# Kateridge/TransMF_AD

Measured on AMD Instinct MI355X. Metric: volume-pairs/sec fwd+bwd(+Adam), 96^3 MRI+PET batch=8 per GPU, higher is better.
Workload: dtype f32

## Files before the change

transmf_ad_amd/csrc/conv3d_wino.hip:

```cpp
#include <type_traits>
#include "tmf_device.h"

namespace {

constexpr int TD = 4, TH = 8, TW = 8;
constexpr int CK = 8;
constexpr int NTHR = 512;
constexpr int GROUPS = 768, SLOTS = 2 * GROUPS;
constexpr int RAW_BYTES = SLOTS * 16;
constexpr int NDMA = SLOTS / NTHR;
constexpr int B_OFF = 2 * RAW_BYTES;
constexpr int B_BYTES = 8 * 8 * 64 * 16;
constexpr int EX_FLOATS = 8 * 8 * 2 * 64 * 4;
constexpr int RED_OFF = EX_FLOATS;
constexpr int LDS_FLOATS = RED_OFF + 8 * 32 * 2;
constexpr size_t LDS_BYTES = (size_t)LDS_FLOATS * 4;
static_assert(B_OFF + B_BYTES <= EX_FLOATS * 4, "LDS carving");

__device__ __forceinline__ constexpr int ogd(int dd) { return (dd & 1) * 384 + (dd >> 1) * 32; }
__device__ __forceinline__ constexpr int ogh(int i) { return (i & 1) * 192 + (i >> 1) * 6; }
__device__ __forceinline__ constexpr int ogw(int k) { return (k & 1) * 96 + (k >> 1); }

#ifdef TMF_WINO_TRACE
__device__ long long g_wino_blocks[8192 * 4];
// ... 863 lines not shown
constexpr int WX_SLOTS = 3072, WX_REAL = 360 * 8, WZ_SLOTS = 1024;
constexpr int WBUF_BYTES = (WX_SLOTS + WZ_SLOTS) * 16;
constexpr int WZ_OFF = WX_SLOTS * 4;
constexpr size_t WG_LDS_BYTES = 2 * (size_t)WBUF_BYTES;

__global__ __launch_bounds__(NTHR) void conv3d_wino_wgrad_kernel(
    const float* __restrict__ x, const float* __restrict__ dz, float* __restrict__ partial,
    int D, int H, int W, int Cin, int Cout, int tilesD, int tilesH, int tilesW, int nbricks, int per_split, int ncob) {
    extern __shared__ __attribute__((aligned(16))) float smem[];
    const unsigned lds0 = (unsigned)(size_t)(__attribute__((address_space(3))) const void*)smem;
    const int tid = threadIdx.x;
    const int lane = tid & 63;
    const int wave = __builtin_amdgcn_readfirstlane(tid >> 6);
    const int l31 = lane & 31, hsel = lane >> 5;
    const int split = blockIdx.x, blk = blockIdx.y;
    const int ci0 = (blk / ncob) * 32, co0 = (blk % ncob) * 32;
    const int st0 = split * per_split;
    const int st1 = st0 + per_split < nbricks ? st0 + per_split : nbricks;
    constexpr int OOB = (int)0x80000000u;

    int relx[6], pcx[6], relz[2], pcz[2];
#pragma unroll
    for (int q = 0; q < 6; ++q) {
        const int e = (q * 8 + wave) * 64 + lane, v = e >> 3, piece = e & 7;
        const int hd = v / 60, hh = (v / 10) % 6, hw = v % 10;
        relx[q] = (((hd - 1) * H + (hh - 1)) * W + (hw - 1)) * Cin * 4 + piece * 16;
        pcx[q] = e < WX_REAL ? (hd | (hh << 8) | (hw << 16)) : -1;
    }
#pragma unroll
    for (int q = 0; q < 2; ++q) {
        const int e = (q * 8 + wave) * 64 + lane, v = e >> 3, piece = e & 7;
        const int od = v >> 5, oh = (v >> 3) & 3, ow = v & 7;
        relz[q] = ((od * H + oh) * W + ow) * Cout * 4 + piece * 16;
        pcz[q] = od | (oh << 8) | (ow << 16);
    }
    auto stage = [&](int st) {
        int t = st;
        const int bw = t % tilesW; t /= tilesW;
        const int bh = t % tilesH; t /= tilesH;
        const int bd = t % tilesD;
        const int b = t / tilesD;
        const int d0 = bd * 4, h0 = bh * 4, w0 = bw * 8;
        const i32x4 xr = make_rsrc(x + (size_t)b * D * H * W * Cin, (unsigned)(D * H * W * Cin * 4));
        const i32x4 zr = make_rsrc(dz + (size_t)b * D * H * W * Cout, (unsigned)(D * H * W * Cout * 4));
        const int xbase = ((d0 * H + h0) * W + w0) * Cin * 4 + ci0 * 4, zbase = ((d0 * H + h0) * W + w0) * Cout * 4 + co0 * 4;
        const unsigned base = lds0 + ((st - st0) & 1) * WBUF_BYTES + wave * 1024;
#pragma unroll
        for (int q = 0; q < 6; ++q) {
            const int hd = pcx[q] & 255, hh = (pcx[q] >> 8) & 255, hw = (pcx[q] >> 16) & 255;
            const bool ok = pcx[q] >= 0 && (unsigned)(d0 - 1 + hd) < (unsigned)D && (unsigned)(h0 - 1 + hh) < (unsigned)H &&
                            (unsigned)(w0 - 1 + hw) < (unsigned)W;
            blds16(ok ? relx[q] + xbase : OOB, xr, 0, base + q * 8192);
        }
#pragma unroll
        for (int q = 0; q < 2; ++q) {
            const int od = pcz[q] & 255, oh = (pcz[q] >> 8) & 255, ow = (pcz[q] >> 16) & 255;
            const bool ok = d0 + od < D && h0 + oh < H && w0 + ow < W;
            blds16(ok ? relz[q] + zbase : OOB, zr, 0, base + WX_SLOTS * 16 + q * 8192);
        }
    };

    const int mpd = wave >> 1, mhh = wave & 1;
    const int da = mpd == 0 ? 0 : (mpd == 2 ? 2 : 1);
    const int db = mpd == 0 ? 2 : (mpd == 1 ? 2 : (mpd == 2 ? 1 : 3));
    const float sgn = mpd == 1 ? 1.f : -1.f;
    const int ik = mhh == 0 ? 2 : 1, ia = mhh == 0 ? 0 : 2, ib = mhh == 0 ? 1 : 3;
    const float c1 = mhh == 0 ? 1.f : -1.f;
    const float ca = mpd == 3 ? 0.f : 1.f, cb = mpd == 0 ? 0.f : (mpd == 1 ? 1.f : -1.f);
    const float e0 = mhh == 0 ? 0.f : -1.f, f0 = mhh == 0 ? 1.f : 0.f, f1 = mhh == 0 ? 1.f : -1.f;
    const int lx = l31 + hsel * 64;
    auto xrow = [&](int dd, int i) { return lx + (dd * 60 + i * 10) * 32; };
    const int rka = xrow(da, ik), rkb = xrow(db, ik), raa = xrow(da, ia), rab = xrow(db, ia), rba = xrow(da, ib), rbb = xrow(db, ib);
    const int lz = WZ_OFF + l31 + hsel * 64;

    f32x16 acc[8];
#pragma unroll
    for (int q = 0; q < 8; ++q)
#pragma unroll
        for (int r = 0; r < 16; ++r) acc[q][r] = 0.f;

    if (st0 < st1) {
        stage(st0);
        vm_wait<0>();
        __syncthreads();
    }
    for (int st = st0; st < st1; ++st) {
        if (st + 1 < st1) stage(st + 1);
        const float* R = smem + ((st - st0) & 1) * (WBUF_BYTES / 4);
#pragma unroll
        for (int j = 0; j < 8; ++j) {
            const int td = j >> 2, th = (j >> 1) & 1, twb = (j & 1) * 2;
            const int xo = ((2 * td * 6 + 2 * th) * 10 + 2 * twb) * 32, zo = ((2 * td * 4 + 2 * th) * 8 + 2 * twb) * 32;
            auto wrow = [&](int pa, int pb, float (&wv)[4]) {
                float tv[4];
#pragma unroll
                for (int k = 0; k < 4; ++k) tv[k] = R[pa + xo + k * 32] + sgn * R[pb + xo + k * 32];
                wv[0] = tv[0] - tv[2]; wv[1] = tv[1] + tv[2]; wv[2] = tv[2] - tv[1]; wv[3] = tv[1] - tv[3];
            };
            float wk[4], A0[4], A1[4];
            wrow(rka, rkb, wk);
            wrow(raa, rab, A0);
            wrow(rba, rbb, A1);
#pragma unroll
            for (int k = 0; k < 4; ++k) {
                A0[k] = A0[k] - wk[k];
                A1[k] = c1 * A1[k] + wk[k];
            }
            float u[2][2];
#pragma unroll
            for (int wo = 0; wo < 2; ++wo) {
                float zd[2];
#pragma unroll
                for (int ho = 0; ho < 2; ++ho)
                    zd[ho] = ca * R[lz + zo + ((0 * 4 + ho) * 8 + wo) * 32] + cb * R[lz + zo + ((1 * 4 + ho) * 8 + wo) * 32];
                u[0][wo] = zd[0] + e0 * zd[1];
                u[1][wo] = f0 * zd[0] + f1 * zd[1];
            }
#pragma unroll
            for (int phl = 0; phl < 2; ++phl) {
                const float b0 = u[phl][0], b1 = u[phl][0] + u[phl][1], b2 = u[phl][0] - u[phl][1], b3 = -u[phl][1];
                const float* Ap = phl == 0 ? A0 : A1;
                acc[phl * 4 + 0] = __builtin_amdgcn_mfma_f32_32x32x2f32(Ap[0], b0, acc[phl * 4 + 0], 0, 0, 0);
                acc[phl * 4 + 1] = __builtin_amdgcn_mfma_f32_32x32x2f32(Ap[1], b1, acc[phl * 4 + 1], 0, 0, 0);
                acc[phl * 4 + 2] = __builtin_amdgcn_mfma_f32_32x32x2f32(Ap[2], b2, acc[phl * 4 + 2], 0, 0, 0);
                acc[phl * 4 + 3] = __builtin_amdgcn_mfma_f32_32x32x2f32(Ap[3], b3, acc[phl * 4 + 3], 0, 0, 0);
            }
        }
        vm_wait<0>();
        __syncthreads();
    }

    float* out = partial + (((size_t)split * gridDim.y + blk) * 64 + (mpd * 16 + mhh * 8)) * 1024;
#pragma unroll
    for (int q = 0; q < 8; ++q)
#pragma unroll
        for (int r = 0; r < 16; ++r)
            out[q * 1024 + ((r & 3) + 8 * (r >> 2) + 4 * hsel) * 32 + l31] = acc[q][r];
}

template <int C, int PAIR = 2>
__device__ __forceinline__ f32x2 lds_pair(unsigned base_even, unsigned base_odd) {
    f32x2 d;
    asm volatile("ds_read2st64_b32 %0, %1 offset0:%2 offset1:%3" : "=v"(d) : "v"((C & 1) ? base_odd : base_even), "n"(C >> 1), "n"((C >> 1) + PAIR));
    return d;
}
__device__ __forceinline__ void lds_wait() { asm volatile("s_waitcnt lgkmcnt(0)" ::: "memory"); }
template <int N, typename F>
__device__ __forceinline__ void static_for(F&& f) {
    if constexpr (N > 0) {
        static_for<N - 1>(f);
        f(std::integral_constant<int, N - 1>{});
    }
}
constexpr int WPN = 256;
template <int GEOM> struct WGeomP {
    static constexpr int ROWW = GEOM == 0 ? 10 : 12, PLANE = 6 * ROWW, PAIR = GEOM == 0 ? 2 : 3, BW = GEOM == 0 ? 8 : 4, BS = GEOM == 0 ? 1 : 2;
    static constexpr int XREAL = 36 * ROWW * 8;
    static constexpr int XDMA = (XREAL + 4 * 64 - 1) / (4 * 64);
    static constexpr int XSLOTS = XDMA * WPN;
    static constexpr int BUF_BYTES = (XSLOTS + WZ_SLOTS) * 16;
    static constexpr size_t LDS_BYTES = 2 * (size_t)BUF_BYTES;
};
constexpr int WP_ZDMA = WZ_SLOTS / WPN;

template <int GEOM>
__global__ __launch_bounds__(WPN) void conv3d_wino_wgrad_p_kernel(
    const float* __restrict__ x, const float* __restrict__ dz, float* __restrict__ partial,
    int B, int D, int H, int W, int Cin, int Cout, int tilesD, int tilesH, int tilesW, int nbricks, int per_split, int ncob) {
    using WG = WGeomP<GEOM>;
    constexpr int WP_XDMA = WG::XDMA, WX_SLOTS = WG::XSLOTS, WX_REAL = WG::XREAL, WBUF_BYTES = WG::BUF_BYTES;
    constexpr int ROWW = WG::ROWW, PLANE = WG::PLANE, PAIR = WG::PAIR;
    extern __shared__ __attribute__((aligned(16))) float smem[];
    const unsigned lds0 = (unsigned)(size_t)(__attribute__((address_space(3))) const void*)smem;
    const int tid = threadIdx.x;
    const int lane = tid & 63;
    const int wave = __builtin_amdgcn_readfirstlane(tid >> 6);
    const int l31 = lane & 31, hsel = lane >> 5;
    const int split = xcd_contiguous(blockIdx.x, gridDim.x), blk = blockIdx.y;
    const int ci0 = (blk / ncob) * 32, co0 = (blk % ncob) * 32;
    const int st0 = split * per_split;
    const int st1 = st0 + per_split < nbricks ? st0 + per_split : nbricks;
    constexpr int OOB = (int)0x80000000u;

    int relx[WP_XDMA], mx[WP_XDMA], relz[WP_ZDMA], mz[WP_ZDMA];
#pragma unroll
    for (int q = 0; q < WP_XDMA; ++q) {
        const int e = (q * 4 + wave) * 64 + lane, v = e >> 3, piece = e & 7;
        const int hd = v / PLANE, hh = (v / ROWW) % 6, hr = v % ROWW, s_ = GEOM == 0 ? 0 : hr / 6, hw = GEOM == 0 ? hr : hr % 6;
        relx[q] = (((s_ * D + hd) * H + hh) * W + hw) * Cin * 4 + piece * 16;
        mx[q] = e < WX_REAL ? (1 << hd) | (1 << (8 + hh)) | (1 << (16 + hw)) | (1 << (26 + s_)) : (1 << 30);
    }
#pragma unroll
    for (int q = 0; q < WP_ZDMA; ++q) {
        const int e = (q * 4 + wave) * 64 + lane, v = e >> 3, piece = e & 7;
        const int od = v >> 5, oh = (v >> 3) & 3, s_ = GEOM == 0 ? 0 : (v >> 2) & 1, ow = GEOM == 0 ? v & 7 : v & 3;
        relz[q] = (((s_ * D + od) * H + oh) * W + ow) * Cout * 4 + piece * 16;
        mz[q] = (1 << od) | (1 << (8 + oh)) | (1 << (16 + ow)) | (1 << (26 + s_));
    }
    int sbw = 0, sbh = 0, sbd = 0, sb = 0;
    auto stage_first = [&](int st) {
        int t = st;
        sbw = t % tilesW; t /= tilesW;
        sbh = t % tilesH; t /= tilesH;
        sbd = t % tilesD;
        sb = t / tilesD;
    };
    auto stage_next = [&]() {
        if (++sbw == tilesW) { sbw = 0; if (++sbh == tilesH) { sbh = 0; if (++sbd == tilesD) { sbd = 0; ++sb; } } }
    };
    i32x4 s_xr, s_zr;
    int s_xcorner = 0, s_zcorner = 0, s_vmx = 0, s_vmz = 0;
    unsigned s_base = 0;
    auto stage_setup = [&](int buf) {
        const int b = sb * WG::BS, d0 = sbd * 4, h0 = sbh * 4, w0 = sbw * WG::BW;
        const int ns = B - b < WG::BS ? B - b : WG::BS;
        s_xr = make_rsrc(x + (size_t)b * D * H * W * Cin, (unsigned)(ns * D * H * W * Cin * 4));
        s_zr = make_rsrc(dz + (size_t)b * D * H * W * Cout, (unsigned)(ns * D * H * W * Cout * 4));
        s_xcorner = (((d0 - 1) * H + (h0 - 1)) * W + (w0 - 1)) * Cin * 4 + ci0 * 4;
        s_zcorner = ((d0 * H + h0) * W + w0) * Cout * 4 + co0 * 4;
        auto range = [](int lo, int hi) { return ((1 << hi) - 1) & ~((1 << lo) - 1); };
        auto mn = [](int a, int b_) { return a < b_ ? a : b_; };
        s_vmx = range(d0 == 0 ? 1 : 0, mn(6, D - d0 + 1)) | (range(h0 == 0 ? 1 : 0, mn(6, H - h0 + 1)) << 8) |
                (range(w0 == 0 ? 1 : 0, mn(WG::BW + 2, W - w0 + 1)) << 16) | (range(0, ns) << 26);
        s_vmz = range(0, mn(4, D - d0)) | (range(0, mn(4, H - h0)) << 8) | (range(0, mn(WG::BW, W - w0)) << 16) | (range(0, ns) << 26);
        s_base = lds0 + buf * WBUF_BYTES + wave * 1024;
    };
    auto stage_part = [&](int part) {
        if (P_ABL & 4) return;
#pragma unroll
        for (int q = 0; q < WP_XDMA; ++q)
            if (q * 3 / WP_XDMA == part) blds16((mx[q] & s_vmx) == mx[q] ? relx[q] + s_xcorner : OOB, s_xr, 0, s_base + q * 4096);
#pragma unroll
        for (int q = 0; q < WP_ZDMA; ++q)
            if (3 == part) blds16((mz[q] & s_vmz) == mz[q] ? relz[q] + s_zcorner : OOB, s_zr, 0, s_base + WX_SLOTS * 16 + q * 4096);
    };
    auto stage_issue = [&](int buf) {
        stage_setup(buf);
#pragma unroll
        for (int i = 0; i < 4; ++i) stage_part(i);
    };

    const int da = wave == 0 ? 0 : (wave == 2 ? 2 : 1);
    const int db = wave == 0 ? 2 : (wave == 1 ? 2 : (wave == 2 ? 1 : 3));
    const float sgn = wave == 1 ? 1.f : -1.f;
    const f32x2 s2 = {sgn, sgn};
    const float cz = wave == 1 ? 1.f : (wave == 2 ? -1.f : 0.f);
    const f32x2 cz2 = {cz, cz};
    const unsigned zfirst = wave == 3 ? 4 * 8 * 32 * 4 : 0;
    const unsigned lx = lds0 + (2 * hsel * 32 + l31) * 4;
    const unsigned xa0 = lx + da * PLANE * 128, xb0 = lx + db * PLANE * 128, zz0 = lx + WX_SLOTS * 16;
    f32x2 A[16], Bv[16];
#if P_ABL & 1
    for (int i = 0; i < 16; ++i) { A[i] = f32x2{(float)tid, 1.f}; Bv[i] = f32x2{(float)lane, 2.f}; }
#endif
    f32x2 u1[4], u2[4], zd[2][2];
    f32x16 acc[16];
#pragma unroll
    for (int q = 0; q < 16; ++q)
#pragma unroll
        for (int r = 0; r < 16; ++r) acc[q][r] = 0.f;

    auto pin4 = [](f32x2& a, f32x2& b, f32x2& c, f32x2& d) { asm volatile("" : "+v"(a), "+v"(b), "+v"(c), "+v"(d)); };
    f32x2 ra[4], rb[4];
    auto row_issue = [&](unsigned ea, unsigned eb, auto c_c) {
        constexpr int Cb = decltype(c_c)::value;
        static_for<4>([&](auto k_c) {
            constexpr int K = decltype(k_c)::value;
            ra[K] = lds_pair<Cb + K, PAIR>(ea, ea + 128);
            rb[K] = lds_pair<Cb + K, PAIR>(eb, eb + 128);
        });
    };
    auto row_finish = [&](f32x2 (&u)[4]) {
        lds_wait();
        pin4(ra[0], ra[1], ra[2], ra[3]);
        pin4(rb[0], rb[1], rb[2], rb[3]);
        pk_row4(u, ra, rb, s2);
    };
    auto zrows = [&](f32x2 ya0, f32x2 ya1, int pha, f32x2 yb0, f32x2 yb1, int phb) {
        Bv[pha * 4 + 0] = ya0; Bv[pha * 4 + 3] = ya1; Bv[phb * 4 + 0] = yb0; Bv[phb * 4 + 3] = yb1;
        pk_z2(Bv[pha * 4 + 1], Bv[pha * 4 + 2], Bv[phb * 4 + 1], Bv[phb * 4 + 2], ya0, ya1, yb0, yb1);
    };
    f32x2 yq[2][2][2];
    f32x2 v0[4];
    auto T1 = [&](int par, auto step_c, int part) {
        constexpr int STEP = decltype(step_c)::value, TDs = STEP >> 1, THs = STEP & 1;
        if (P_ABL & 1) return;
        const unsigned off = par * WBUF_BYTES;
        if (part == 0) {
            row_issue(xa0 + off, xb0 + off, std::integral_constant<int, (2 * TDs) * PLANE + (2 * THs + 1) * ROWW>{});
            static_for<2>([&](auto ho_c) {
                static_for<2>([&](auto wo_c) {
                    constexpr int HO = decltype(ho_c)::value, WO = decltype(wo_c)::value;
                    constexpr int C0 = ((2 * TDs + 0) * 4 + (2 * THs + HO)) * 8 + WO, C1 = ((2 * TDs + 1) * 4 + (2 * THs + HO)) * 8 + WO;
                    yq[0][HO][WO] = lds_pair<C0>(zz0 + zfirst + off, zz0 + zfirst + off + 128);
                    yq[1][HO][WO] = lds_pair<C1>(zz0 + off, zz0 + off + 128);
                });
            });
        } else if (part == 1) {
            row_finish(u1);
            pin4(yq[0][0][0], yq[0][0][1], yq[0][1][0], yq[0][1][1]);
            pin4(yq[1][0][0], yq[1][0][1], yq[1][1][0], yq[1][1][1]);
            row_issue(xa0 + off, xb0 + off, std::integral_constant<int, (2 * TDs) * PLANE + (2 * THs + 2) * ROWW>{});
#pragma unroll
            for (int ho = 0; ho < 2; ++ho)
#pragma unroll
                for (int wo = 0; wo < 2; ++wo) zd[ho][wo] = pk_fma(cz2, yq[1][ho][wo], yq[0][ho][wo]);
            {
                f32x2 zs0, zdf0, zs1, zdf1;
                pk_z2(zs0, zdf0, zs1, zdf1, zd[0][0], zd[1][0], zd[0][1], zd[1][1]);
                zrows(zs0, zs1, 1, zdf0, zdf1, 2);
            }
            pin4(u1[0], u1[1], u1[2], u1[3]);
            pin4(Bv[4], Bv[5], Bv[6], Bv[7]); pin4(Bv[8], Bv[9], Bv[10], Bv[11]);
        } else {
            row_finish(u2);
            {
                f32x2 sm[4], df[4];
                pk_addsub4(sm, df, u2, u1);
#pragma unroll
                for (int k = 0; k < 4; ++k) { A[4 + k] = sm[k]; A[8 + k] = df[k]; }
            }
            pin4(A[4], A[5], A[6], A[7]); pin4(A[8], A[9], A[10], A[11]);
        }
    };
    auto T2 = [&](int par, auto step_c, int part) {
        constexpr int STEP = decltype(step_c)::value, TDs = STEP >> 1, THs = STEP & 1;
        if (P_ABL & 1) return;
        const unsigned off = par * WBUF_BYTES;
        if (part == 0) {
            row_issue(xa0 + off, xb0 + off, std::integral_constant<int, (2 * TDs) * PLANE + (2 * THs + 0) * ROWW>{});
            zrows(zd[0][0], zd[0][1], 0, zd[1][0], zd[1][1], 3);
            pin4(Bv[0], Bv[1], Bv[2], Bv[3]); pin4(Bv[12], Bv[13], Bv[14], Bv[15]);
        } else if (part == 1) {
            row_finish(v0);
            row_issue(xa0 + off, xb0 + off, std::integral_constant<int, (2 * TDs) * PLANE + (2 * THs + 3) * ROWW>{});
            {
                f32x2 d[4];
                pk_sub4(d, v0, u2);
#pragma unroll
                for (int k = 0; k < 4; ++k) A[k] = d[k];
            }
            pin4(A[0], A[1], A[2], A[3]);
        } else {
            row_finish(v0);
            {
                f32x2 d[4];
                pk_sub4(d, u1, v0);
#pragma unroll
                for (int k = 0; k < 4; ++k) A[12 + k] = d[k];
            }
            pin4(A[12], A[13], A[14], A[15]);
        }
    };
    auto mfma_g = [&](int pha, int phb, int g) {
        const int k0 = g == 2 ? 0 : 2 * g, k1 = g == 2 ? 4 : 2 * g + 2, s0 = g == 2 ? 1 : 0;
#pragma unroll
        for (int k = k0; k < k1; ++k) {
#if P_ABL & 16
            acc[pha * 4 + k][s0] += A[pha * 4 + k][s0] * Bv[pha * 4 + k][s0]; acc[phb * 4 + k][s0] += A[phb * 4 + k][s0] * Bv[phb * 4 + k][s0];
#else
            acc[pha * 4 + k] = __builtin_amdgcn_mfma_f32_32x32x2f32(A[pha * 4 + k][s0], Bv[pha * 4 + k][s0], acc[pha * 4 + k], 0, 0, 0);
            acc[phb * 4 + k] = __builtin_amdgcn_mfma_f32_32x32x2f32(A[phb * 4 + k][s0], Bv[phb * 4 + k][s0], acc[phb * 4 + k], 0, 0, 0);
#endif
        }
    };

    if (st0 < st1) {
        stage_first(st0);
        stage_issue(0);
        if (st0 + 1 < st1) { stage_next(); stage_issue(1); }
        vm_wait<0>();
        __syncthreads();
#pragma unroll
        for (int g = 0; g < 3; ++g) T1(0, std::integral_constant<int, 0>{}, g);
        bool pend = false;
        for (int st = st0; st < st1; ++st) {
            const int par = (st - st0) & 1;
            static_for<4>([&](auto step_c) {
                constexpr int STEP = decltype(step_c)::value;
                __builtin_amdgcn_sched_barrier(0);
                if (STEP < 2 && pend) { stage_part(1 + 2 * STEP); if (STEP == 1) pend = false; }
#pragma unroll
                for (int g = 0; g < 3; ++g) {
                    __builtin_amdgcn_sched_barrier(0);
                    T2(par, step_c, g);
                    mfma_g(1, 2, g);
                }
                __builtin_amdgcn_sched_barrier(0);
                if (STEP == 3) {
                    vm_wait<0>();
                    __syncthreads();
                    if (st + 2 < st1) { stage_next(); stage_setup(par); stage_part(0); pend = true; }
                }
                if (STEP == 0 && pend) stage_part(2);
#pragma unroll
                for (int g = 0; g < 3; ++g) {
                    __builtin_amdgcn_sched_barrier(0);
                    T1(STEP < 3 ? par : par ^ 1, std::integral_constant<int, (STEP + 1) & 3>{}, g);
                    mfma_g(0, 3, g);
                }
                __builtin_amdgcn_sched_barrier(0);
            });
        }
    }

    __syncthreads();
    float* slab = partial + (size_t)split * 27 * Cin * Cout + (size_t)ci0 * Cout + co0 + l31;
    auto gt3 = [](float u0, float u1, float u2, float u3, float (&o)[3]) {
        const float sm = u1 + u2, df = u1 - u2;
        o[0] = u0 + 0.5f * sm; o[1] = 0.5f * df; o[2] = 0.5f * sm - u3;
    };
#pragma unroll
    for (int half = 0; half < 2; ++half) {
#pragma unroll
        for (int rr = 0; rr < 8; ++rr) {
            const int r = half * 8 + rr;
            float t[4][3], v[3][3];
#pragma unroll
            for (int ph = 0; ph < 4; ++ph)
                gt3(acc_read(acc[ph * 4 + 0][r]), acc_read(acc[ph * 4 + 1][r]), acc_read(acc[ph * 4 + 2][r]), acc_read(acc[ph * 4 + 3][r]), t[ph]);
#pragma unroll
            for (int j = 0; j < 3; ++j) {
                float o[3];
                gt3(t[0][j], t[1][j], t[2][j], t[3][j], o);
                v[0][j] = o[0]; v[1][j] = o[1]; v[2][j] = o[2];
            }
#pragma unroll
            for (int i = 0; i < 3; ++i)
#pragma unroll
                for (int j = 0; j < 3; ++j) smem[((wave * 8 + rr) * 9 + i * 3 + j) * 64 + lane] = v[i][j];
            __builtin_amdgcn_sched_barrier(0);
        }
        __syncthreads();
#pragma unroll
        for (int q = 0; q < 18; ++q) {
            const int e = wave * 18 + q, rr = e / 9, ij = e % 9;
            float V[4], o[3];
#pragma unroll
            for (int pd = 0; pd < 4; ++pd) V[pd] = smem[((pd * 8 + rr) * 9 + ij) * 64 + lane];
            gt3(V[0], V[1], V[2], V[3], o);
            const int r = half * 8 + rr, ci = (r & 3) + 8 * (r >> 2) + 4 * hsel;
#pragma unroll
            for (int kd = 0; kd < 3; ++kd) slab[((size_t)(kd * 9 + ij) * Cin + ci) * Cout] = o[kd];
        }
        __syncthreads();
    }
}

__global__ __launch_bounds__(256) void wino_wgrad_finish_kernel(const float* __restrict__ du, float* __restrict__ dw,
                                                                int cin, int cout, int ncob, int dw_ref) {
    const int e = blockIdx.x * 256 + threadIdx.x;
    if (e >= cin * cout) return;
    const int co = e % cout, ci = e / cout;
    const int blk = (ci / 32) * ncob + co / 32;
    const float* src = du + (size_t)blk * 64 * 1024 + (ci % 32) * 32 + (co % 32);
    double u[4][4][4];
#pragma unroll
    for (int p = 0; p < 4; ++p)
#pragma unroll
        for (int q = 0; q < 4; ++q)
#pragma unroll
            for (int r = 0; r < 4; ++r) u[p][q][r] = (double)src[((p * 4 + q) * 4 + r) * 1024];
    auto GT = [](double u0, double u1, double u2, double u3, int a) {
        return a == 0 ? u0 + 0.5 * (u1 + u2) : (a == 1 ? 0.5 * (u1 - u2) : 0.5 * (u1 + u2) + u3);
    };
    double t1[3][4][4], t2[3][3][4];
#pragma unroll
    for (int a = 0; a < 3; ++a)
#pragma unroll
        for (int q = 0; q < 4; ++q)
#pragma unroll
            for (int r = 0; r < 4; ++r) t1[a][q][r] = GT(u[0][q][r], u[1][q][r], u[2][q][r], u[3][q][r], a);
#pragma unroll
    for (int a = 0; a < 3; ++a)
#pragma unroll
        for (int bq = 0; bq < 3; ++bq)
#pragma unroll
            for (int r = 0; r < 4; ++r) t2[a][bq][r] = GT(t1[a][0][r], t1[a][1][r], t1[a][2][r], t1[a][3][r], bq);
#pragma unroll
    for (int a = 0; a < 3; ++a)
#pragma unroll
        for (int bq = 0; bq < 3; ++bq)
#pragma unroll
            for (int c = 0; c < 3; ++c) {
                const float v = (float)GT(t2[a][bq][0], t2[a][bq][1], t2[a][bq][2], t2[a][bq][3], c);
                const int tap = (a * 3 + bq) * 3 + c;
                if (dw_ref) dw[((size_t)co * cin + ci) * 27 + tap] = v;
                else dw[((size_t)tap * cin + ci) * cout + co] = v;
            }
}

int wino_p_mode();
struct WinoWgPlan { int geom, tilesD, tilesH, tilesW, nbricks, nblk, ncob, nsplit, per; };
WinoWgPlan plan_wino_wgrad(int B, int D, int H, int W, int cin, int cout) {
    WinoWgPlan p;
    p.tilesD = tmf_cdiv(D, 4); p.tilesH = tmf_cdiv(H, 4); p.tilesW = tmf_cdiv(W, 8);
    p.nbricks = B * p.tilesD * p.tilesH * p.tilesW;
    p.geom = 0;
    const long two = 2L * D * H * W * (cin > cout ? cin : cout) * 4;
    const int nb1 = tmf_cdiv(B, 2) * p.tilesD * p.tilesH * tmf_cdiv(W, 4);
    if (wino_p_mode() && nb1 < p.nbricks && two < (1L << 31)) {
        p.geom = 1;
        p.tilesW = tmf_cdiv(W, 4);
        p.nbricks = nb1;
// ... 397 lines not shown
```

transmf_ad_amd/csrc/conv3d_winox.hip:

```cpp
#include <type_traits>
#include "tmf_device.h"

#ifndef X_PF
#define X_PF 2
#endif
#ifndef X_NGFAST
#define X_NGFAST 1
#endif
#ifndef X_SKEW
#define X_SKEW 0
#endif
#ifndef X_RB
#define X_RB 0
#endif
#ifndef X_ABL
#define X_ABL 0
#endif

namespace {

#ifdef TMF_WINOX_TRACE
__device__ long long g_winox_phases[8 * 64];
#define XTR(i) do { __builtin_amdgcn_sched_barrier(0); if (blockIdx.x == 77 && it == 1 && lane == 0) xtr_lds[wave * 64 + (i)] = (long long)__builtin_readcyclecounter(); __builtin_amdgcn_sched_barrier(0); } while (0)
#define XTRC(i) XTR((i) + 20 * (c & 1))
#else
#define XTR(i)
#define XTRC(i)
#endif

constexpr int XN = 512;
constexpr int XCK = 16;
constexpr int BD = 4, BH = 8, BW = 8;
constexpr int CP = 96, SD = 32, SH = 6;
constexpr int SLOTS_G = 16 * CP;
constexpr int RAWB = SLOTS_G * 16;
constexpr int XDMA = SLOTS_G / XN;
constexpr int TS = 68;
constexpr int EX_OFF = 2 * RAWB;
constexpr int EX_BYTES = 8 * 32 * TS * 4;
constexpr int RED_OFF = EX_OFF + EX_BYTES;
constexpr int PLAN_OFF = RED_OFF + 2 * 64 * 33 * 4 + 64;
constexpr int TAB_OFF = PLAN_OFF + 9 * XN * 4;
#ifdef TMF_WINOX_TRACE
constexpr int TAB = 96;
#else
constexpr int TAB = 256;
#endif
constexpr size_t X_LDS_BYTES = (size_t)TAB_OFF + 256 * 32;
static_assert(EX_OFF + EX_BYTES >= 4 * RAWB && X_LDS_BYTES <= 160 * 1024, "LDS carving");

__device__ __forceinline__ void pin3(i32x4& a, i32x4& b, i32x4& c) { asm volatile("" : "+v"(a), "+v"(b), "+v"(c)); }
__device__ __forceinline__ void wg_barrier() {
    asm volatile("s_waitcnt lgkmcnt(0)\n\ts_barrier" ::: "memory");
}

__device__ __forceinline__ void wg_barrier_if(int flag) {
    asm volatile("s_cmp_eq_u32 %0, 0\n\ts_cbranch_scc1 .LWGB%=\n\ts_waitcnt lgkmcnt(0)\n\ts_barrier\n.LWGB%=:" ::"s"(__builtin_amdgcn_readfirstlane(flag)) : "memory", "scc");
}

__device__ __forceinline__ void split8(const float (&y0)[4], const float (&y1)[4], i32x4& H, i32x4& M, i32x4& L) {
#pragma unroll
    for (int j = 0; j < 4; ++j) {
        const float a = j < 2 ? y0[2 * j] : y1[2 * j - 4], b = j < 2 ? y0[2 * j + 1] : y1[2 * j - 3];
        const unsigned ua = __builtin_bit_cast(unsigned, a), ub = __builtin_bit_cast(unsigned, b);
        const float ra = a - __builtin_bit_cast(float, ua & 0xFFFF0000u), rb = b - __builtin_bit_cast(float, ub & 0xFFFF0000u);
        const unsigned va = __builtin_bit_cast(unsigned, ra), vb = __builtin_bit_cast(unsigned, rb);
        const float la = ra - __builtin_bit_cast(float, va & 0xFFFF0000u), lb = rb - __builtin_bit_cast(float, vb & 0xFFFF0000u);
        H[j] = (int)__builtin_amdgcn_perm(ub, ua, 0x07060302u);
        M[j] = (int)__builtin_amdgcn_perm(vb, va, 0x07060302u);
        L[j] = (int)__builtin_amdgcn_perm(__builtin_bit_cast(unsigned, lb), __builtin_bit_cast(unsigned, la), 0x07060302u);
    }
}
__device__ __forceinline__ f32x16 mfma_bf16(i32x4 a, i32x4 b, f32x16 c) {
    return __builtin_amdgcn_mfma_f32_32x32x16_bf16(__builtin_bit_cast(tmf_bf16x8, a), __builtin_bit_cast(tmf_bf16x8, b), c, 0, 0, 0);
}

template <int MODE>
__global__ __launch_bounds__(XN) void conv3d_winox_kernel(
    const float* __restrict__ x, const unsigned short* __restrict__ u3, float* __restrict__ z, float* __restrict__ stat_partial,
    int B, int D, int H, int W, int Cin, int Cout, int tilesD, int tilesH, int tilesW, int nbricks, int item0, int nitems,
    int stat_rows, int stat_accum, const float* __restrict__ aff_scale = nullptr, const float* __restrict__ aff_shift = nullptr,
    float slope = 0.f, int swap = 0) {
    const int sd = swap ? W : H * W, sh = swap ? D * W : W;
    constexpr bool STATS = MODE == 1;
    constexpr bool AFFINE = MODE >= 2, POOL = MODE == 3;
    constexpr int EPI_STORES = POOL ? 1 : 4;
    extern __shared__ __attribute__((aligned(16))) float smem[];
    float* ex = smem + EX_OFF / 4;
    float* red = smem + RED_OFF / 4;
    i32x4* tab = reinterpret_cast<i32x4*>(smem + TAB_OFF / 4);
#ifdef TMF_WINOX_TRACE
    long long* xtr_lds = reinterpret_cast<long long*>(smem + TAB_OFF / 4 + TAB * 8);
    for (int i = threadIdx.x; i < 512; i += XN) xtr_lds[i] = 0;
#endif
    const unsigned lds0 = (unsigned)(size_t)(__attribute__((address_space(3))) const void*)smem;
    const int tid = threadIdx.x;
    const int lane = tid & 63;
    const int wave = __builtin_amdgcn_readfirstlane(tid >> 6);
    const int l31 = lane & 31, hsel = lane >> 5;
    const int mpd = wave >> 1, mhh = wave & 1;
    const int late = (X_SKEW && wave >= 4) ? 1 : 0, early = late ^ 1;
    const int nchunk = Cin / XCK;
    constexpr int OOB = (int)0x80000000u;

    const int G = gridDim.x;
    const int jb = xcd_contiguous(blockIdx.x, G);
    const int my_items = jb < nitems ? (nitems - jb + G - 1) / G : 0;
    if (my_items == 0) return;
    for (int i = tid; i < my_items; i += XN) {
        const int item = item0 + jb + i * G;
#if X_NGFAST
        const int ngroups = Cout >> 5;
        int t = item / ngroups;
        const int ng = item - t * ngroups;
#else
        const int ng = item / nbricks;
        int t = item - ng * nbricks;
#endif
        const int bw = t % tilesW; t /= tilesW;
        const int bh = t % tilesH; t /= tilesH;
        const int bd = t % tilesD;
        const int b0 = t / tilesD;
        tab[2 * i] = i32x4{0, ng, b0, bd | (bh << 10) | (bw << 20)};
        const int d0 = bd * BD, h0 = bh * BH, w0 = bw * BW;
        auto range = [](int lo, int hi) { return ((1 << hi) - 1) & ~((1 << lo) - 1); };
        auto mn = [](int a, int b_) { return a < b_ ? a : b_; };
        tab[2 * i + 1] = i32x4{((d0 - 1) * sd + (h0 - 1) * sh + (w0 - 1)) * Cin * 4,
                               range(d0 == 0 ? 1 : 0, mn(BD + 2, D - d0 + 1)) | (range(h0 == 0 ? 1 : 0, mn(BH + 2, H - h0 + 1)) << 6) |
                                   (range(w0 == 0 ? 1 : 0, mn(BW + 2, W - w0 + 1)) << 16), 0, 0};
    }
    __syncthreads();

    int* plan = reinterpret_cast<int*>(smem + PLAN_OFF / 4) + tid;
#pragma unroll
    for (int q = 0; q < XDMA; ++q) {
        const int e = (q * 8 + wave) * 64 + lane, gg = e >> 1, par = gg / CP, g = gg % CP;
        const int a_ = g / 32, bb = (g % 32) / 6, c_ = (g % 32) % 6;
        const bool real = bb < 5 && c_ < 5;
        const int hd = 2 * a_ + (par >> 2), hh = 2 * bb + ((par >> 1) & 1), hw = 2 * c_ + (par & 1);
        const int quad = (e & 1) ^ (bb & 1);
        plan[q * XN] = ((hd * sd + hh * sh + hw) * Cin + quad * 4) * 4;
        plan[(3 + q) * XN] = real ? (1 << hd) | (1 << (6 + hh)) | (1 << (16 + hw)) : (1 << 30);
    }
    i32x4 xr = make_rsrc(x, 0);
    int dm_i = 0, dm_c = 0;
    auto dma_plan = [&](int i) {
        int corner = 0, vm = 0;
        if (i >= 0) {
            const i32x4 e1 = tab[2 * i + 1];
            const int b = __builtin_amdgcn_readfirstlane(tab[2 * i][2]);
            corner = __builtin_amdgcn_readfirstlane(e1[0]);
            vm = __builtin_amdgcn_readfirstlane(e1[1]);
            xr = make_rsrc(x + (size_t)b * D * H * W * Cin, (unsigned)(D * H * W * Cin * 4));
        }
#pragma unroll
        for (int q = 0; q < XDMA; ++q) {
            const int m = plan[(3 + q) * XN];
            plan[(6 + q) * XN] = (m & vm) == m ? plan[q * XN] + corner : OOB;
        }
    };
    auto dma_part = [&](int pr, int part) {
        const unsigned base = lds0 + pr * 2 * RAWB + wave * 1024 + part * 8192;
        const int ho = plan[(6 + part) * XN];
        if (!(X_ABL & 4)) {
            blds16_uniform(ho, xr, dm_c * (XCK * 4), base);
            blds16_uniform(ho, xr, dm_c * (XCK * 4) + 32, base + RAWB);
// ... 57 lines not shown
        for (int k = 0; k < 4; ++k) {
#pragma unroll
            for (int e = 0; e < 4; ++e) {
                const float tx = ax[k][e] + sgn * bx[k][e], tk = ak[k][e] + sgn * bk[k][e];
                T[k][e] = GA ? tx - tk : c1 * tx + tk;
            }
        }
#pragma unroll
        for (int e = 0; e < 4; ++e) {
            Y[0][e] = T[0][e] - T[2][e]; Y[1][e] = T[1][e] + T[2][e]; Y[2][e] = T[2][e] - T[1][e]; Y[3][e] = T[1][e] - T[3][e];
        }
    };

    f32x16 acc[8];

    const int r_td = wave >> 2, r_th = wave & 3;
    auto lane_now = [&]() { int l = lane; asm volatile("" : "+v"(l)); return l; };
    int st_n0 = -1;
    unsigned st_seen = 0;
    auto stat_zero = [&]() {
        const int le = lane_now();
        float* red_l = red + (wave * 8 + (le >> 3)) * 33 + 4 * (le & 7);
#pragma unroll
        for (int e = 0; e < 4; ++e) { red_l[e] = 0.f; red_l[64 * 33 + e] = 0.f; }
    };
    auto stat_flush = [&]() {
        __syncthreads();
        if (tid < 256) {
            const int part = tid & 3, ch = (tid >> 2) & 31, which = tid >> 7;
            float a = 0.f;
#pragma unroll
            for (int m = 0; m < 16; ++m) a += red[(which * 64 + part * 16 + m) * 33 + ch];
            a += __builtin_bit_cast(float, __builtin_amdgcn_mov_dpp(__builtin_bit_cast(int, a), 0xB1, 0xF, 0xF, true));
            a += __builtin_bit_cast(float, __builtin_amdgcn_mov_dpp(__builtin_bit_cast(int, a), 0x4E, 0xF, 0xF, true));
            if (part == 0) {
                float* dst = stat_partial + ((size_t)blockIdx.x * 2 + which) * Cout + st_n0 + ch;
                *dst = (stat_accum || ((st_seen >> (st_n0 >> 5)) & 1)) ? *dst + a : a;
            }
        }
        st_seen |= 1u << (st_n0 >> 5);
        __syncthreads();
        stat_zero();
    };
    if (STATS) stat_zero();

    int ci_n0 = __builtin_amdgcn_readfirstlane(tab[0][1]) * 32;
    dma_plan(0);
#pragma unroll
    for (int i = 0; i < XDMA; ++i) dma_part(0, i);
    load_b(0, 0, 0, ci_n0);
    if (X_PF == 2) load_b(1, 1, 0, ci_n0);
    vm_wait<0>();
    __syncthreads();

    int g = 0;
    for (int it = 0; it < my_items; ++it) {
        const i32x4 ce = tab[2 * it];
        const int b = __builtin_amdgcn_readfirstlane(ce[2]);
        const int cpk = __builtin_amdgcn_readfirstlane(ce[3]);
        const int d0 = (cpk & 1023) * BD, h0 = ((cpk >> 10) & 1023) * BH, w0 = (cpk >> 20) * BW;
        const int n0 = ci_n0;
        auto chunk = [&](int c, auto first_c) {
            constexpr bool FIRST = decltype(first_c)::value;
            const int pr = g & 1;
            const float* R0 = smem + pr * (2 * RAWB / 4);
            const float* R1 = R0 + RAWB / 4;
            int nc = c + 1, n0n = n0;
            if (nc == nchunk) {
                nc = 0;
                n0n = __builtin_amdgcn_readfirstlane(tab[2 * (it + 1 < my_items ? it + 1 : it)][1]) * 32;
                ci_n0 = n0n;
            }
            float Y0[4][4], Y1[4][4];
            auto position = [&](auto q8_c, const float (&y0)[4], const float (&y1)[4]) {
                constexpr int q8 = decltype(q8_c)::value;
                if (q8 + X_PF < 8) load_b((q8 + X_PF) & 3, q8 + X_PF, c, n0);
                else load_b((q8 + X_PF) & 3, q8 + X_PF - 8, nc, n0n);
                constexpr int cnt = 3 * X_PF + (q8 < X_PF ? ((X_ABL & 4) ? 0 : 6) + (FIRST && !(X_ABL & 8) ? EPI_STORES : 0) : 0);
                vm_wait<cnt>();
                pin3(Bq[q8 & 3][0], Bq[q8 & 3][1], Bq[q8 & 3][2]);
                i32x4 vh, vm_, vl;
                if (X_ABL & 32) {
                    vh = i32x4{__builtin_bit_cast(int, y0[0]), __builtin_bit_cast(int, y0[1]), __builtin_bit_cast(int, y0[2]), __builtin_bit_cast(int, y0[3])};
                    vm_ = i32x4{__builtin_bit_cast(int, y1[0]), __builtin_bit_cast(int, y1[1]), __builtin_bit_cast(int, y1[2]), __builtin_bit_cast(int, y1[3])};
                    vl = vh;
                } else
                    split8(y0, y1, vh, vm_, vl);
                const f32x16 zero = {0.f, 0.f, 0.f, 0.f, 0.f, 0.f, 0.f, 0.f, 0.f, 0.f, 0.f, 0.f, 0.f, 0.f, 0.f, 0.f};
                const i32x4 wh = Bq[q8 & 3][0], wm = Bq[q8 & 3][1], wl = Bq[q8 & 3][2];
#if X_ABL & 16
                f32x16 a = FIRST ? zero : acc[q8];
#pragma unroll
                for (int e = 0; e < 4; ++e) a[e] += __builtin_bit_cast(float, wh[e] ^ vl[e] ^ wl[e] ^ vh[e] ^ wm[e] ^ vm_[e]);
                acc[q8] = a;
#else
                f32x16 a = mfma_bf16(wh, vl, FIRST ? zero : acc[q8]);
                a = mfma_bf16(wl, vh, a);
                a = mfma_bf16(wm, vm_, a);
                a = mfma_bf16(wh, vm_, a);
                a = mfma_bf16(wm, vh, a);
                acc[q8] = mfma_bf16(wh, vh, a);
#endif
            };
            XTRC(0);
            __builtin_amdgcn_sched_barrier(0);
#pragma unroll
            for (int i = 0; i < XDMA; ++i) dma_part(pr ^ 1, i);
            group_rows(R0, raa, rab, std::true_type{}, Y0);
            group_rows(R1, raa, rab, std::true_type{}, Y1);
            __builtin_amdgcn_sched_barrier(0);
            XTRC(1);
            wg_barrier_if(late);
            position(std::integral_constant<int, 0>{}, Y0[0], Y1[0]);
            position(std::integral_constant<int, 1>{}, Y0[1], Y1[1]);
            position(std::integral_constant<int, 2>{}, Y0[2], Y1[2]);
            position(std::integral_constant<int, 3>{}, Y0[3], Y1[3]);
            XTRC(2);
            __builtin_amdgcn_sched_barrier(0);
            if (X_SKEW) wg_barrier_if(early);
            group_rows(R0, rba, rbb, std::false_type{}, Y0);
            group_rows(R1, rba, rbb, std::false_type{}, Y1);
            __builtin_amdgcn_sched_barrier(0);
            XTRC(3);
            wg_barrier_if(late);
            position(std::integral_constant<int, 4>{}, Y0[0], Y1[0]);
            position(std::integral_constant<int, 5>{}, Y0[1], Y1[1]);
            position(std::integral_constant<int, 6>{}, Y0[2], Y1[2]);
            position(std::integral_constant<int, 7>{}, Y0[3], Y1[3]);
            __builtin_amdgcn_sched_barrier(0);
            XTRC(4);
            wg_barrier_if(early);
            XTRC(5);
            ++g;
        };
        chunk(0, std::true_type{});
        for (int c = 1; c < nchunk; ++c) chunk(c, std::false_type{});

#if X_ABL & 8
        {
            float sm = 0.f;
#pragma unroll
            for (int q = 0; q < 8; ++q) sm += acc[q][0] + acc[q][7];
            if (sm == 12345.678f) z[tid] = sm + (float)(b + d0 + h0 + w0 + n0);
            wg_barrier();
            continue;
        }
#endif
        f32x4 P1[4][2];
        const int le = lane_now();
        const int cq = le & 7, rwo = (le >> 3) & 1, vq = le >> 4, r_tw = vq;
        const int st_lane = ((2 * r_td * sd + 2 * r_th * sh + 2 * r_tw + rwo) * Cout + 4 * cq) * 4;
        float* red_l = red + (wave * 8 + (le >> 3)) * 33 + 4 * cq;
        float* exw = ex + (wave * 32 + (le & 31)) * TS + 4 * (le >> 5);
#pragma unroll
        for (int j = 0; j < 4; ++j) {
            f32x4 y[2][2];
#pragma unroll
            for (int phl = 0; phl < 2; ++phl) {
                f32x4 m[4];
#pragma unroll
                for (int pw = 0; pw < 4; ++pw)
                    m[pw] = f32x4{acc[phl * 4 + pw][4 * j], acc[phl * 4 + pw][4 * j + 1], acc[phl * 4 + pw][4 * j + 2], acc[phl * 4 + pw][4 * j + 3]};
                y[phl][0] = (m[0] + m[1]) + m[2];
                y[phl][1] = (m[1] - m[2]) - m[3];
            }
#pragma unroll
            for (int wo = 0; wo < 2; ++wo) {
                const f32x4 sum = y[0][wo] + y[1][wo];
                const f32x4 p0 = mhh == 0 ? sum : y[0][wo];
                P1[j][wo] = mhh == 0 ? y[1][wo] : sum;
                *reinterpret_cast<f32x4*>(&exw[wo * 32 + 8 * j]) = p0;
            }
        }
        XTR(40);
        const int OD = D / 2, OH = H / 2, OW = W / 2;
        float* zb = z + (size_t)b * (POOL ? OD * OH * OW : D * H * W) * Cout;
        const __amdgpu_buffer_rsrc_t zr = __builtin_amdgcn_make_buffer_rsrc(zb, 0, (POOL ? OD * OH * OW : D * H * W) * Cout * 4, 0x00020000);
        const bool full = d0 + BD <= D && h0 + BH <= H && w0 + BW <= W;
        if (STATS && stat_partial != nullptr && st_n0 != n0) {
            if (st_n0 >= 0) stat_flush();
            st_n0 = n0;
        }
        if (AFFINE && st_n0 != n0) {
            __syncthreads();
            if (tid < 64) red[tid] = tid < 32 ? aff_scale[n0 + tid] : aff_shift[n0 + tid - 32];
            __syncthreads();
            st_n0 = n0;
        }
        f32x4 a_sc = {1.f, 1.f, 1.f, 1.f}, a_sh = {0.f, 0.f, 0.f, 0.f}, pmax = {0.f, 0.f, 0.f, 0.f};
        if (AFFINE) {
            a_sc = *reinterpret_cast<const f32x4*>(&red[4 * cq]);
            a_sh = *reinterpret_cast<const f32x4*>(&red[32 + 4 * cq]);
        }
        const int gd0 = d0 + 2 * r_td, gh0 = h0 + 2 * r_th, gw = w0 + 2 * r_tw + rwo;
        const int st_item = ((d0 * sd + h0 * sh + w0) * Cout + n0) * 4;
        const float* exr = ex + (4 * wave + vq) * TS + rwo * 32 + 4 * cq;
        auto pass = [&](int ho) {
            wg_barrier();
            XTR(41 + 4 * ho);
            f32x4 S[4];
#pragma unroll
            for (int pd = 0; pd < 4; ++pd) {
                const f32x4 lo = *reinterpret_cast<const f32x4*>(&exr[(2 * pd) * 32 * TS]);
                const f32x4 hi = *reinterpret_cast<const f32x4*>(&exr[(2 * pd + 1) * 32 * TS]);
                S[pd] = ho == 0 ? lo + hi : lo - hi;
            }
            f32x4 o[2];
            o[0] = (S[0] + S[1]) + S[2];
            o[1] = (S[1] - S[2]) - S[3];
            const int gh = gh0 + ho;
            if (AFFINE) {
#pragma unroll
                for (int dd = 0; dd < 2; ++dd)
#pragma unroll
                    for (int e = 0; e < 4; ++e) {
                        const float yv = o[dd][e] * a_sc[e] + a_sh[e];
                        o[dd][e] = yv > 0.f ? yv : yv * slope;
                    }
            }
            if (POOL) {
#pragma unroll
                for (int e = 0; e < 4; ++e) {
                    const float v = fmaxf(o[0][e], o[1][e]);
                    pmax[e] = ho == 0 ? v : fmaxf(pmax[e], v);
                }
                if (ho == 1) {
                    f32x4 m;
#pragma unroll
                    for (int e = 0; e < 4; ++e) {
                        float other;
                        asm volatile("s_nop 1\n\tv_mov_b32_dpp %0, %1 row_ror:8 row_mask:0xf bank_mask:0xf" : "=&v"(other) : "v"(pmax[e]));
                        m[e] = fmaxf(pmax[e], other);
                    }
                    const int od = (d0 >> 1) + r_td, oh = (h0 >> 1) + r_th, ow = (w0 >> 1) + r_tw;
                    const bool okp = rwo == 0 && od < OD && oh < OH && ow < OW;
                    const int osd = swap ? OW : OH * OW, osh = swap ? OD * OW : OW;
                    const int voff = ((r_td * osd + r_th * osh + r_tw) * Cout + 4 * cq) * 4;
                    __builtin_amdgcn_raw_buffer_store_b128(__builtin_bit_cast(tmf_u32x4, m), zr, okp ? voff : OOB,
                                                           (((d0 >> 1) * osd + (h0 >> 1) * osh + (w0 >> 1)) * Cout + n0) * 4, 0);
                    store_guard();
                }
                return;
            }
#pragma unroll
            for (int dd = 0; dd < 2; ++dd) {
                const bool ok = full || (gd0 + dd < D && gh < H && gw < W);
                __builtin_amdgcn_raw_buffer_store_b128(__builtin_bit_cast(tmf_u32x4, o[dd]), zr, ok ? st_lane : OOB,
                                                       st_item + (dd * sd + ho * sh) * Cout * 4, 0);
                store_guard();
                if (STATS) {
#pragma unroll
                    for (int e = 0; e < 4; ++e) {
                        const float v = ok ? o[dd][e] : 0.f;
                        red_l[e] += v;
                        red_l[64 * 33 + e] += v * v;
                    }
                }
            }
        };
        pass(0);
        XTR(42);
        wg_barrier();
        XTR(43);
#pragma unroll
        for (int j = 0; j < 4; ++j)
#pragma unroll
            for (int wo = 0; wo < 2; ++wo) *reinterpret_cast<f32x4*>(&exw[wo * 32 + 8 * j]) = P1[j][wo];
        XTR(44);
        pass(1);
        XTR(46);
        wg_barrier();
        XTR(47);
    }
    vm_wait<0>();
#ifdef TMF_WINOX_TRACE
    __syncthreads();
    if (blockIdx.x == 77) for (int i = threadIdx.x; i < 512; i += XN) g_winox_phases[i] = xtr_lds[i];
#endif
    if constexpr (STATS) {
        if (stat_partial != nullptr) {
            if (st_n0 >= 0) stat_flush();
            if (!stat_accum) {
                for (int ng = 0; ng < Cout / 32; ++ng)
                    if (!((st_seen >> ng) & 1) && tid < 64) stat_partial[((size_t)blockIdx.x * 2 + (tid >> 5)) * Cout + ng * 32 + (tid & 31)] = 0.f;
                if (blockIdx.x == 0)
                    for (int i = (int)gridDim.x * 2 * Cout + tid; i < stat_rows * 2 * Cout; i += XN) stat_partial[i] = 0.f;
            }
        }
    }
}

}
#ifdef TMF_WINOX_TRACE
extern "C" int tmf_winox_trace_read(long long* phases) {
    return (int)hipMemcpyFromSymbol(phases, HIP_SYMBOL(g_winox_phases), sizeof(long long) * 8 * 64);
}
#endif
int tmf_winox_takes(int B, int D, int H, int W, int cin, int cout, int geom) {
    return tmf_opt(TMF_OPT_WINO_X) && geom == 0 && cin % 32 == 0 && cout % 32 == 0 && cout <= 1024;
}

long tmf_winox_items(int D, int H, int W, int* swap) {
    const long t_n = (long)tmf_cdiv(D, BD) * tmf_cdiv(H, BH) * tmf_cdiv(W, BW);
    const long t_s = (long)tmf_cdiv(H, BD) * tmf_cdiv(D, BH) * tmf_cdiv(W, BW);
    const int sw = tmf_opt(TMF_OPT_WINOX_SWAP) && t_s < t_n ? 1 : 0;
    if (swap) *swap = sw;
    return sw ? t_s : t_n;
}

int tmf_winox_first_grid(long nitems, int ncu) {
    const long per_launch = (long)ncu * TAB;
    return tmf_wino_window_grid(nitems < per_launch ? nitems : per_launch, ncu, 1);
}

int tmf_winox_launch(const char* what, const float* x, const unsigned short* u3, float* z, float* stat_partial, int B, int Dt, int Ht,
                     int W, int cin, int cout, int ncu, hipStream_t stream, const float* scale, const float* shift, float slope, int pool) {
    int swap = 0;
    tmf_winox_items(Dt, Ht, W, &swap);
    const int D = swap ? Ht : Dt, H = swap ? Dt : Ht;
    const int tilesD = tmf_cdiv(D, BD), tilesH = tmf_cdiv(H, BH), tilesW = tmf_cdiv(W, BW);
    TMF_REQUIRE(tilesD < 1024 && tilesH < 1024 && tilesW < 1024, TMF_E_SHAPE, "%s: more than 1023 bricks along one axis", what);
    TMF_REQUIRE((long)D * H * W * (cin > cout ? cin : cout) < (1L << 29), TMF_E_SHAPE,
                "%s: one sample exceeds 2^29 elements (32-bit byte offsets)", what);
    TMF_REQUIRE((long)64 * cin * cout * 6 < (1L << 31), TMF_E_SHAPE, "%s: weight tensor exceeds 2^31 bytes", what);
    const long nbricks = (long)B * tilesD * tilesH * tilesW;
    const long nitems = nbricks * (cout / 32);
    TMF_REQUIRE(nitems < (1L << 30), TMF_E_SHAPE, "%s: too many bricks", what);
    int rc;
    auto launch = [&](auto k, int mode_stats) -> int {
        if ((rc = tmf_allow_lds(k, X_LDS_BYTES, what))) return rc;
        const long per_launch = (long)ncu * TAB;
        for (long i0 = 0; i0 < nitems; i0 += per_launch) {
            const long n = nitems - i0 < per_launch ? nitems - i0 : per_launch;
            const int grid = tmf_wino_window_grid(n, ncu, 1);
            hipLaunchKernelGGL(k, dim3(grid), dim3(XN), X_LDS_BYTES, stream, x, u3, z, stat_partial, B, D, H, W, cin, cout,
                               tilesD, tilesH, tilesW, (int)nbricks, (int)i0, (int)n, ncu, i0 > 0 ? 1 : 0, scale, shift, slope, swap);
            if ((rc = tmf_launch_result(what))) return rc;
        }
        return TMF_OK;
    };
    if (scale != nullptr) return pool == TMF_POOL_MAX2 ? launch(conv3d_winox_kernel<3>, 3) : launch(conv3d_winox_kernel<2>, 2);
    if (stat_partial != nullptr) return launch(conv3d_winox_kernel<1>, 1);
    return launch(conv3d_winox_kernel<0>, 0);
}
```

Baseline: 1014.

## Reuse input rows across Winograd wgrad steps, use FMA role blend, register stats

In the Winograd weight-gradient kernel, rows already transformed in the previous H-step (THs==0) are carried in registers (k2, u1) into the THs==1 step, so two of the four LDS row reads per step are skipped. In the fused output kernel, the per-lane select between sum and passthrough is replaced by FMAs with 0/1 coefficients. BatchNorm statistics are accumulated in registers across both passes instead of read-modify-writing LDS on every element. The register carry adds register pressure and relies on the step ordering matching the carried values.

```diff
diff --git a/transmf_ad_amd/csrc/conv3d_wino.hip b/transmf_ad_amd/csrc/conv3d_wino.hip
--- a/transmf_ad_amd/csrc/conv3d_wino.hip
+++ b/transmf_ad_amd/csrc/conv3d_wino.hip
@@ -1039,6 +1039,9 @@
         f(std::integral_constant<int, N - 1>{});
     }
 }
+#ifndef W_REUSE
+#define W_REUSE 1
+#endif
 constexpr int WPN = 256;
 template <int GEOM> struct WGeomP {
     static constexpr int ROWW = GEOM == 0 ? 10 : 12, PLANE = 6 * ROWW, PAIR = GEOM == 0 ? 2 : 3, BW = GEOM == 0 ? 8 : 4, BS = GEOM == 0 ? 1 : 2;
@@ -1169,12 +1172,14 @@
     };
     f32x2 yq[2][2][2];
     f32x2 v0[4];
+    f32x2 k2[4];
     auto T1 = [&](int par, auto step_c, int part) {
         constexpr int STEP = decltype(step_c)::value, TDs = STEP >> 1, THs = STEP & 1;
         if (P_ABL & 1) return;
         const unsigned off = par * WBUF_BYTES;
+        constexpr bool CARRY = W_REUSE && THs == 1;
         if (part == 0) {
-            row_issue(xa0 + off, xb0 + off, std::integral_constant<int, (2 * TDs) * PLANE + (2 * THs + 1) * ROWW>{});
+            row_issue(xa0 + off, xb0 + off, std::integral_constant<int, (2 * TDs) * PLANE + (2 * THs + (CARRY ? 2 : 1)) * ROWW>{});
             static_for<2>([&](auto ho_c) {
                 static_for<2>([&](auto wo_c) {
                     constexpr int HO = decltype(ho_c)::value, WO = decltype(wo_c)::value;
@@ -1184,10 +1189,11 @@
                 });
             });
         } else if (part == 1) {
-            row_finish(u1);
+            if (CARRY) lds_wait();
+            else row_finish(u1);
             pin4(yq[0][0][0], yq[0][0][1], yq[0][1][0], yq[0][1][1]);
             pin4(yq[1][0][0], yq[1][0][1], yq[1][1][0], yq[1][1][1]);
-            row_issue(xa0 + off, xb0 + off, std::integral_constant<int, (2 * TDs) * PLANE + (2 * THs + 2) * ROWW>{});
+            if (!CARRY) row_issue(xa0 + off, xb0 + off, std::integral_constant<int, (2 * TDs) * PLANE + (2 * THs + 2) * ROWW>{});
 #pragma unroll
             for (int ho = 0; ho < 2; ++ho)
 #pragma unroll
@@ -1214,16 +1220,20 @@
         constexpr int STEP = decltype(step_c)::value, TDs = STEP >> 1, THs = STEP & 1;
         if (P_ABL & 1) return;
         const unsigned off = par * WBUF_BYTES;
+        constexpr bool CARRY = W_REUSE && THs == 1;
         if (part == 0) {
-            row_issue(xa0 + off, xb0 + off, std::integral_constant<int, (2 * TDs) * PLANE + (2 * THs + 0) * ROWW>{});
+            row_issue(xa0 + off, xb0 + off, std::integral_constant<int, (2 * TDs) * PLANE + (2 * THs + (CARRY ? 3 : 0)) * ROWW>{});
             zrows(zd[0][0], zd[0][1], 0, zd[1][0], zd[1][1], 3);
             pin4(Bv[0], Bv[1], Bv[2], Bv[3]); pin4(Bv[12], Bv[13], Bv[14], Bv[15]);
         } else if (part == 1) {
-            row_finish(v0);
-            row_issue(xa0 + off, xb0 + off, std::integral_constant<int, (2 * TDs) * PLANE + (2 * THs + 3) * ROWW>{});
+            if (!CARRY) {
+                row_finish(v0);
+                row_issue(xa0 + off, xb0 + off, std::integral_constant<int, (2 * TDs) * PLANE + (2 * THs + 3) * ROWW>{});
+            }
             {
                 f32x2 d[4];
-                pk_sub4(d, v0, u2);
+                if constexpr (CARRY) pk_sub4(d, k2, u2);
+                else pk_sub4(d, v0, u2);
 #pragma unroll
                 for (int k = 0; k < 4; ++k) A[k] = d[k];
             }
@@ -1237,6 +1247,10 @@
                 for (int k = 0; k < 4; ++k) A[12 + k] = d[k];
             }
             pin4(A[12], A[13], A[14], A[15]);
+            if (W_REUSE && THs == 0) {
+#pragma unroll
+                for (int k = 0; k < 4; ++k) { k2[k] = u2[k]; u1[k] = v0[k]; }
+            }
         }
     };
     auto mfma_g = [&](int pha, int phb, int g) {
diff --git a/transmf_ad_amd/csrc/conv3d_winox.hip b/transmf_ad_amd/csrc/conv3d_winox.hip
--- a/transmf_ad_amd/csrc/conv3d_winox.hip
+++ b/transmf_ad_amd/csrc/conv3d_winox.hip
@@ -12,6 +12,12 @@
 #endif
 #ifndef X_RB
 #define X_RB 0
+#endif
+#ifndef X_ROLE_FMA
+#define X_ROLE_FMA 1
+#endif
+#ifndef X_STAT_REG
+#define X_STAT_REG 1
 #endif
 #ifndef X_ABL
 #define X_ABL 0
@@ -375,6 +381,9 @@
         const int st_lane = ((2 * r_td * sd + 2 * r_th * sh + 2 * r_tw + rwo) * Cout + 4 * cq) * 4;
         float* red_l = red + (wave * 8 + (le >> 3)) * 33 + 4 * cq;
         float* exw = ex + (wave * 32 + (le & 31)) * TS + 4 * (le >> 5);
+#if X_ROLE_FMA
+        const float rc0 = mhh == 0 ? 1.f : 0.f, rc1 = mhh == 0 ? 0.f : 1.f;
+#endif
 #pragma unroll
         for (int j = 0; j < 4; ++j) {
             f32x4 y[2][2];
@@ -389,9 +398,18 @@
             }
 #pragma unroll
             for (int wo = 0; wo < 2; ++wo) {
+#if X_ROLE_FMA
+                f32x4 p0;
+#pragma unroll
+                for (int e = 0; e < 4; ++e) {
+                    p0[e] = __builtin_fmaf(rc0, y[1][wo][e], y[0][wo][e]);
+                    P1[j][wo][e] = __builtin_fmaf(rc1, y[0][wo][e], y[1][wo][e]);
+                }
+#else
                 const f32x4 sum = y[0][wo] + y[1][wo];
                 const f32x4 p0 = mhh == 0 ? sum : y[0][wo];
                 P1[j][wo] = mhh == 0 ? y[1][wo] : sum;
+#endif
                 *reinterpret_cast<f32x4*>(&exw[wo * 32 + 8 * j]) = p0;
             }
         }
@@ -418,6 +436,7 @@
         const int gd0 = d0 + 2 * r_td, gh0 = h0 + 2 * r_th, gw = w0 + 2 * r_tw + rwo;
         const int st_item = ((d0 * sd + h0 * sh + w0) * Cout + n0) * 4;
         const float* exr = ex + (4 * wave + vq) * TS + rwo * 32 + 4 * cq;
+        float st_s[4] = {0.f, 0.f, 0.f, 0.f}, st_q[4] = {0.f, 0.f, 0.f, 0.f};
         auto pass = [&](int ho) {
             wg_barrier();
             XTR(41 + 4 * ho);
@@ -475,12 +494,21 @@
 #pragma unroll
                     for (int e = 0; e < 4; ++e) {
                         const float v = ok ? o[dd][e] : 0.f;
+#if X_STAT_REG
+                        st_s[e] += v;
+                        st_q[e] += v * v;
+#else
                         red_l[e] += v;
                         red_l[64 * 33 + e] += v * v;
+#endif
                     }
                 }
             }
         };
+        if (STATS && X_STAT_REG) {
+#pragma unroll
+            for (int e = 0; e < 4; ++e) { st_s[e] = red_l[e]; st_q[e] = red_l[64 * 33 + e]; }
+        }
         pass(0);
         XTR(42);
         wg_barrier();
@@ -491,6 +519,10 @@
             for (int wo = 0; wo < 2; ++wo) *reinterpret_cast<f32x4*>(&exw[wo * 32 + 8 * j]) = P1[j][wo];
         XTR(44);
         pass(1);
+        if (STATS && X_STAT_REG) {
+#pragma unroll
+            for (int e = 0; e < 4; ++e) { red_l[e] = st_s[e]; red_l[64 * 33 + e] = st_q[e]; }
+        }
         XTR(46);
         wg_barrier();
         XTR(47);
```

Result: faster. 1053, median of 6 (+3.9%).
